# ctu-vras/trajectory_optimization

Hardware: AMD Instinct MI355X
Metric: point-visibility evals/sec (fwd+bwd) (higher is better)
Workload: dtype f32

## Files before the change

trajectory_optimization_amd/csrc/traj_kernels.hip:

```cpp
#include <algorithm>
#include <atomic>
#include <cstdlib>
#include <type_traits>

#include "common.hpp"
#include "opt_step.hpp"
#include "profile.hpp"

#define TO_SLOT 256
#define TO_TIE_CAP 7
#define TO_BWD_NSUM 14
#define TO_SP_THREADS 1024
#define TO_SP_WAVES (TO_SP_THREADS / 64)
#define TO_CBIT_STRIDE 16
#define TO_PROBE_MAXFW 1024
#define TO_SP_MAXW 1024
#define TO_PL_SHARDS 64
#define TO_PL_STRIDE 32

#ifdef TOHIP_STAMPS
#define TO_STAMP_BLOCKS 1024
#define TO_STAMP_N 12
enum { TO_STAMP_PROBE = 0, TO_STAMP_CULL, TO_STAMP_SPARSE, TO_STAMP_PAIRS, TO_STAMP_FINISH, TO_STAMP_KERNELS };
__device__ unsigned long long g_stamps[TO_STAMP_KERNELS][TO_STAMP_BLOCKS][TO_STAMP_N];
// ... 265 lines not shown
                const f2 p = vis_p_pk(r, k, f2{px[j], px[j + 1]}, f2{py[j], py[j + 1]}, f2{pz[j], pz[j + 1]}) *
                             f2{occ_one(occ, occw, v, (int64_t)sj0 * cv.sample_step), sj1 < cv.nsamples ? occ_one(occ, occw, v, (int64_t)sj1 * cv.sample_step) : 1.0f};
                mx = fmaxf(mx, p.x);
                mn = fminf(mn, p.x);
                if (sj1 < cv.nsamples) { mx = fmaxf(mx, p.y); mn = fminf(mn, p.y); }
            }
        }
    }
    for (int s = 32; s > 0; s >>= 1) { mx = fmaxf(mx, __shfl_xor(mx, s)); mn = fminf(mn, __shfl_xor(mn, s)); }
    if ((t & 63) == 0) { smx[t >> 6] = mx; smn[t >> 6] = mn; }
    __syncthreads();
    TO_STAMP(TO_STAMP_PROBE, 2);
    if (t == 0) {
        for (int w = 1; w < TO_PROBE_THREADS / 64; ++w) { mx = fmaxf(mx, smx[w]); mn = fminf(mn, smn[w]); }
        if (!(mn <= mx)) { mx = 0.f; mn = INFINITY; }
        const bool poisoned = cv.hdr[1] != 0;
        if (poisoned) { mx = __builtin_nanf(""); mn = INFINITY; }
        float thr, sthr;
        cull_bound(0.5f * mx, k.inv_var, &thr, &sthr);
        rec[v].Lh = (mn == 0.f && !poisoned) ? 0.49f * mx : 0.f;
        rec[v].L = mx;
        rec[v].U = mn;
        rec[v].thr1 = thr;
        rec[v].sthr1 = sthr;
        rec[v].azero = (mn == 0.f) ? 1.f : 0.f;
        scull[0] = thr; scull[1] = sthr; scull[2] = (mn == 0.f) ? 1.f : 0.f;
        Extrema e;
        e.nmn = -__builtin_bit_cast(int, mn);
        e.mx = __builtin_bit_cast(int, mx);
        e.pad[0] = e.pad[1] = 0;
        ext[v] = e;
        ties[v].nmax = 0;
        ties[v].nmin = 0;
    }
    TO_STAMP(TO_STAMP_PROBE, 3);
    if (!pc.on) return;
    __syncthreads();
    const float thr = scull[0], sthr = scull[1], azero = scull[2], inv_scd = 1.0f / k.scd;
    const int lane = t & 63;
    auto test_word = [&](int w, const float4& b) {
        const int sl = w * 64 + lane;
        const unsigned long long word = __ballot(sl < pc.nslots && tile_live(r.t, r.sp, thr, sthr, azero, b, inv_scd));
        if (lane == 0) pc.live[(int64_t)v * fv_words + w] = word;
    };
#pragma unroll
    for (int i = 0; i < kPre; ++i)
        if ((t >> 6) + i * kWaves < fv_words) test_word((t >> 6) + i * kWaves, tb[i]);
    for (int w0 = (t >> 6) + kPre * kWaves; w0 < fv_words; w0 += kPre * kWaves) {
#pragma unroll
        for (int i = 0; i < kPre; ++i) {
            const int sl = (w0 + i * kWaves) * 64 + lane;
            tb[i] = cv.bounds[sl < pc.nslots ? sl : 0];
        }
#pragma unroll
        for (int i = 0; i < kPre; ++i)
            if (w0 + i * kWaves < fv_words) test_word(w0 + i * kWaves, tb[i]);
    }
    TO_STAMP(TO_STAMP_PROBE, 4);
}


#define TO_P 4

__device__ __forceinline__ bool fold_extrema(Extrema* __restrict__ ext, int v, float mn, float mx, const WayRec& r) {
    bool cand = false;
    if (!(mx < r.Lh)) {
        cand = true;
        const int mxb = __builtin_bit_cast(int, mx);
        if (mxb > __builtin_bit_cast(int, r.L)) atomicMax(&ext[v].mx, mxb);
    }
    const int Ub = __builtin_bit_cast(int, r.U);
    if (Ub != 0) {
        const int mnb = __builtin_bit_cast(int, mn);
        if (mnb < Ub) atomicMax(&ext[v].nmn, -mnb);
    }
    return cand;
}

__device__ __forceinline__ unsigned long long* cbit_word(unsigned long long* cbits, int fv_words, int seg, int w) {
    return cbits + ((int64_t)seg * fv_words + w) * TO_CBIT_STRIDE;
}
__device__ __forceinline__ void mark_candidate(unsigned long long* __restrict__ cbits, int fv_words, int slot, int seg) {
    atomicOr(cbit_word(cbits, fv_words, seg, slot >> 6), 1ull << (slot & 63));
}

#define TO_PD 8
#define TO_DENSE_SGPRS 112
#define TO_DENSE_OCC_SGPRS 112
template <bool OCC>
__global__ void __launch_bounds__(TO_BLOCK)
k_traj_pass1_dense(CloudView cv, const WayRec* __restrict__ rec, int V, int nblk, EvalK k, float2* __restrict__ part,
                   Extrema* __restrict__ ext, unsigned long long* __restrict__ cbits, int fv_words,
                   const uint32_t* __restrict__ occ, int64_t occw, OutInit oi, unsigned long long* __restrict__ stamps) {
    constexpr int P = TO_PD;
    const int lane = threadIdx.x & 63;
    unsigned long long st0 = 0, sr0 = 0;
    if (stamps != nullptr && threadIdx.x == 0) { st0 = __builtin_amdgcn_s_memtime(); sr0 = __builtin_amdgcn_s_memrealtime(); }
    f2 eps2 = pk_splat(k.eps), l2e2 = pk_splat(k.l2e_eps), scd2 = pk_splat(k.scd);
    asm volatile("" : "+v"(eps2), "+v"(l2e2), "+v"(scd2));
    const int64_t total = (int64_t)nblk * V;
    int64_t u = total * blockIdx.x / gridDim.x;
    const int64_t u_end = total * (blockIdx.x + 1) / gridDim.x;
    const int64_t len = u_end - u, q1 = u + 3 * len / 4, q2 = u + 7 * len / 8, q3 = u + 15 * len / 16;
    __builtin_amdgcn_s_setprio(3);
    while (u < u_end) {
        const int pb = (int)(u / V);
        const int v0 = (int)(u - (int64_t)pb * V);
        const int v1 = (int)min((int64_t)V, v0 + (u_end - u));
        const int gthread = pb * TO_BLOCK + threadIdx.x;
        const int64_t base = (int64_t)gthread * P;
        const int slot = gthread >> 5;
        float x[P], y[P], z[P];
        load_points<P>(cv.soa, cv.npad, base, x, y, z);
        if (v0 == 0) { init_outputs(base, oi); init_outputs(base + 4, oi); }
        float2* prow = part + (int64_t)slot * V;
        for (int v = v0; v < v1; ++v) {
            const int64_t uu = u + (v - v0);
            if (uu == q1) __builtin_amdgcn_s_setprio(2);
            if (uu == q2) __builtin_amdgcn_s_setprio(1);
            if (uu == q3) __builtin_amdgcn_s_setprio(0);
            const WayRec& r = rec[v];
            float om[P];
            load_occ<P, OCC>(occ, occw, v, base, om);
            f2 p[P / 2];
#pragma unroll
            for (int i = 0; i < P; i += 2)
                p[i / 2] = vis_p_pk(r, k, f2{x[i], x[i + 1]}, f2{y[i], y[i + 1]}, f2{z[i], z[i + 1]}, eps2, l2e2, scd2) * f2{om[i], om[i + 1]};
            const float m1 = fmaxf(fmaxf(p[0].x, p[0].y), p[1].x), m2 = fmaxf(fmaxf(p[1].y, p[2].x), p[2].y);
            float mx = fmaxf(m2, fmaxf(fmaxf(p[3].x, p[3].y), m1));
            mx = half_max31_nn_fused(mx);
            float mn = 0.f;
            if (__builtin_bit_cast(int, r.U) != 0) {
                mn = fminf(fminf(fminf(p[0].x, p[0].y), fminf(p[1].x, p[1].y)), fminf(fminf(p[2].x, p[2].y), fminf(p[3].x, p[3].y)));
                mn = half_min31_nn_fused(mn);
            }
            if ((lane & 31) == 31) {
                prow[v] = make_float2(mn, mx);
                if (fold_extrema(ext, v, mn, mx, r)) mark_candidate(cbits, fv_words, slot, r.seg);
            }
        }
        u += v1 - v0;
    }
    if (stamps != nullptr && threadIdx.x == 0) {
        stamps[2 * blockIdx.x] = __builtin_amdgcn_s_memtime() - st0;
        stamps[2 * blockIdx.x + 1] = __builtin_amdgcn_s_memrealtime() - sr0;
        unsigned long long* ext_st = stamps + 2 * (int64_t)gridDim.x + 4 * (int64_t)blockIdx.x;
        unsigned hw, xcc;
        asm volatile("s_getreg_b32 %0, hwreg(HW_REG_HW_ID)" : "=s"(hw));
        asm volatile("s_getreg_b32 %0, hwreg(HW_REG_XCC_ID)" : "=s"(xcc));
        ext_st[0] = sr0; ext_st[1] = __builtin_amdgcn_s_memrealtime(); ext_st[2] = hw; ext_st[3] = xcc;
    }
}

__device__ __forceinline__ unsigned long long uniform_u64(unsigned long long v) {
    const unsigned lo = __builtin_amdgcn_readfirstlane((unsigned)v), hi = __builtin_amdgcn_readfirstlane((unsigned)(v >> 32));
    return ((unsigned long long)hi << 32) | lo;
}

#define TO_CULL_LIST 2048
struct CullLds {
    unsigned long long cand[TO_PROBE_MAXFW];
    unsigned long long row[TO_PROBE_MAXFW];
    int pre[TO_PROBE_MAXFW];
    int list[TO_CULL_LIST];
    int mx[2 * TO_SP_WAVES], mn[2 * TO_SP_WAVES];
    int total;
};

__device__ __forceinline__ int cull_select(const CullLds& L, int fv_words, int j, int lane) {
    int lo = 0, hi = fv_words;
    while (hi - lo > 1) {
        const int step = (hi - lo + 63) >> 6;
        const int idx = lo + lane * step;
        const int cnt = __popcll(__ballot(idx < hi && L.pre[idx] <= j));
        lo += (cnt - 1) * step;
        hi = min(hi, lo + step);
    }
    const unsigned long long word = uniform_u64(L.row[lo]);
    const int r = j - L.pre[lo];
    const bool hit = ((word >> lane) & 1ull) && __popcll(word & ((1ull << lane) - 1ull)) == r;
    return lo * 64 + __builtin_ctzll(__ballot(hit));
}

template <bool OCC, int NW>
__global__ void __launch_bounds__(NW * 64)
k_traj_pass1_cull(CloudView cv, const WayRec* __restrict__ rec, int V, EvalK k, float2* __restrict__ part, Extrema* __restrict__ ext,
                  unsigned long long* __restrict__ cbits, int fv_words, const unsigned long long* __restrict__ live,
                  const uint32_t* __restrict__ occ, int64_t occw, OutInit oi) {
    __shared__ CullLds L;
    const int t = threadIdx.x, lane = t & 63, wave = t >> 6;
    const int v = blockIdx.y;
    TO_STAMP(TO_STAMP_CULL, 0);
    for (int w = t; w < fv_words; w += NW * 64) { L.row[w] = live[(int64_t)v * fv_words + w]; L.cand[w] = 0ull; }
    if (oi.lo_zero != nullptr)
        for (int64_t i = (((int64_t)v * gridDim.x + blockIdx.x) * (NW * 64) + t) * 4; i < oi.npad; i += (int64_t)gridDim.y * gridDim.x * (NW * 64) * 4)
            init_outputs(i, oi);
    __syncthreads();
    TO_STAMP(TO_STAMP_CULL, 1);
    if (t < 64) {
        int carry = 0;
        for (int w0 = 0; w0 < fv_words; w0 += 64) {
            const int c = (w0 + lane < fv_words) ? __popcll(L.row[w0 + lane]) : 0;
            int incl = c;
#pragma unroll
            for (int sh = 1; sh < 64; sh <<= 1) {
                const int up = __shfl_up(incl, sh);
                if (lane >= sh) incl += up;
            }
            if (w0 + lane < fv_words) L.pre[w0 + lane] = carry + incl - c;
            carry += __shfl(incl, 63);
        }
        if (lane == 0) L.total = carry;
    }
    __syncthreads();
    const int n = L.total;
    const bool listed = n <= TO_CULL_LIST;
    if (listed) {
        for (int w = wave; w < fv_words; w += NW) {
            const unsigned long long word = L.row[w];
            if ((word >> lane) & 1ull) L.list[L.pre[w] + __popcll(word & ((1ull << lane) - 1ull))] = w * 64 + lane;
        }
        __syncthreads();
    }
    TO_STAMP(TO_STAMP_CULL, 2);
    const int wr = __builtin_amdgcn_readfirstlane((int)(blockIdx.x * NW) + wave), WR = (int)gridDim.x * NW;
    const WayRec& r = rec[v];
    int bmx = __builtin_bit_cast(int, r.L), bmn = __builtin_bit_cast(int, r.U);
    const int half = lane >> 5, nunits = (n + 1) >> 1;
    auto unit_slot = [&](int u) {
        if (listed) return L.list[min(2 * u + half, n - 1)];
        const int s0 = cull_select(L, fv_words, 2 * u, lane), s1 = cull_select(L, fv_words, min(2 * u + 1, n - 1), lane);
        return half ? s1 : s0;
    };
    if (wr < nunits) {
        constexpr int P8 = TO_PD;
        const f2 eps2 = pk_splat(k.eps), l2e2 = pk_splat(k.l2e_eps), scd2 = pk_splat(k.scd);
        auto eval_unit = [&](int u, int cur, const float (&x)[P8], const float (&y)[P8], const float (&z)[P8]) {
            const bool valid = 2 * u + half < n;
            float om[P8];
            load_occ<P8, OCC>(occ, occw, v, (int64_t)cur * TO_SLOT + (lane & 31) * P8, om);
            f2 p[P8 / 2];
#pragma unroll
            for (int i = 0; i < P8; i += 2)
                p[i / 2] = vis_p_pk(r, k, f2{x[i], x[i + 1]}, f2{y[i], y[i + 1]}, f2{z[i], z[i + 1]}, eps2, l2e2, scd2) * f2{om[i], om[i + 1]};
            const float m1 = fmaxf(fmaxf(p[0].x, p[0].y), p[1].x), m2 = fmaxf(fmaxf(p[1].y, p[2].x), p[2].y);
            const float mx = half_max31_nn_fused(fmaxf(m2, fmaxf(fmaxf(p[3].x, p[3].y), m1)));
            float mn = 0.f;
            if (__builtin_bit_cast(int, r.U) != 0) {
                mn = fminf(fminf(fminf(p[0].x, p[0].y), fminf(p[1].x, p[1].y)), fminf(fminf(p[2].x, p[2].y), fminf(p[3].x, p[3].y)));
                mn = half_min31_nn_fused(mn);
            }
            if ((lane & 31) == 31 && valid) {
                part[(int64_t)cur * V + v] = make_float2(mn, mx);
                if (!(mx < r.Lh)) {
                    atomicOr(&L.cand[cur >> 6], 1ull << (cur & 63));
                    bmx = max(bmx, __builtin_bit_cast(int, mx));
                }
                if (__builtin_bit_cast(int, r.U) != 0) bmn = min(bmn, __builtin_bit_cast(int, mn));
            }
        };
        float xa[P8], ya[P8], za[P8], xb[P8], yb[P8], zb[P8];
        int sa = unit_slot(wr), sb = 0;
        load_points<P8>(cv.soa, cv.npad, (int64_t)sa * TO_SLOT + (lane & 31) * P8, xa, ya, za);
        for (int u = wr; u < nunits; u += 2 * WR) {
            const bool more1 = u + WR < nunits, more2 = u + 2 * WR < nunits;
            if (more1) {
                sb = unit_slot(u + WR);
                load_points<P8>(cv.soa, cv.npad, (int64_t)sb * TO_SLOT + (lane & 31) * P8, xb, yb, zb);
            }
            eval_unit(u, sa, xa, ya, za);
            if (!more1) break;
            if (more2) {
                sa = unit_slot(u + 2 * WR);
                load_points<P8>(cv.soa, cv.npad, (int64_t)sa * TO_SLOT + (lane & 31) * P8, xa, ya, za);
            }
            eval_unit(u + WR, sb, xb, yb, zb);
        }
    }
    TO_STAMP(TO_STAMP_CULL, 3);
    if ((lane & 31) == 31) { L.mx[2 * wave + half] = bmx; L.mn[2 * wave + half] = bmn; }
    __syncthreads();
    TO_STAMP(TO_STAMP_CULL, 4);
    if (t == 0) {
        for (int w = 0; w < 2 * NW; ++w) { bmx = max(bmx, L.mx[w]); bmn = min(bmn, L.mn[w]); }
        if (bmx > __builtin_bit_cast(int, r.L)) atomicMax(&ext[v].mx, bmx);
        if (bmn < __builtin_bit_cast(int, r.U)) atomicMax(&ext[v].nmn, -bmn);
    }
    for (int w = t; w < fv_words; w += NW * 64) {
        const unsigned long long word = L.cand[w];
        if (word) atomicOr(cbit_word(cbits, fv_words, r.seg, w), word);
    }
    TO_STAMP(TO_STAMP_CULL, 5);
}


enum { TO_SP_FWD = 0, TO_SP_FUSED = 2 };
#define TO_SP_CW 4
#define TO_SP_STAGE (TO_SP_CW * 64)

struct SparseArgs {
    CloudView cv;
    const WayRec* rec;
    const Extrema* ext;
    EvalK k;
    const float2* part;
    int V, nslots, vwords, fv_words;
    const unsigned long long* cbits;
    const unsigned long long* live;
    int2* plist;
    int* npairs;
    int64_t plcap;
    unsigned long long* fv;
    TieRec* ties;
    float* lo_sum;
    float* minmax;
    const uint32_t* occ;
    int64_t occw;
    const int* toff;
    int n_traj, C;
    float* rewards;
    int prefilled;
    RewardAcc* acc;
    int shift;
    const float* grad_rewards;
    const float* scalars;
    const float* gout;
    float* bpart;
    float* unit;
};

struct __attribute__((aligned(16))) StagedWay {
    float t[3], f0[3], f1[3], f2[3], sp[3];
    float a, invM;
    int v;
    float pad[2];
};
static_assert(sizeof(StagedWay) == 80, "StagedWay is 20 floats");

template <int NW, int SFW>
struct SparseLds {
    unsigned long long sflag[SFW];
    StagedWay stage[TO_SP_STAGE];
    float4 spart[TO_SP_WAVES][64];
    int any[NW];
    int pbase;
};

__device__ __forceinline__ f2 log_odds_pk(const EvalK& k, float a, float invM, f2 p) {
    f2 ph = (p - pk_splat(a)) * pk_splat(invM);
    ph = f2{__builtin_amdgcn_fmed3f(ph.x, 0.5f, k.clip_hi), __builtin_amdgcn_fmed3f(ph.y, 0.5f, k.clip_hi)};
    const f2 om = pk_splat(1.0f) - ph;
    return (f2{to_log2(ph.x), to_log2(ph.y)} - f2{to_log2(om.x), to_log2(om.y)}) * pk_splat(0.693147180559945f);
}

__device__ __forceinline__ void stage_way(const SparseArgs& a, int v, StagedWay& dst) {
    const WayRec& r = a.rec[v];
    StagedWay sw;
    for (int i = 0; i < 3; ++i) { sw.t[i] = r.t[i]; sw.f0[i] = r.f0[i]; sw.f1[i] = r.f1[i]; sw.f2[i] = r.f2[i]; sw.sp[i] = r.sp[i]; }
    float pmax, M;
    load_norm(a.ext[v], sw.a, pmax, M, sw.invM);
    if (!(M > 0.f) || !(sw.invM < INFINITY)) sw.invM = __builtin_nanf("");
    sw.v = v;
    sw.pad[0] = sw.pad[1] = 0.f;
    dst = sw;
}

template <int MODE, bool OCC, int NW, int SFW>
__device__ __forceinline__ void sparse_slot(const SparseArgs& a, int slot, int tr, int acc_line, SparseLds<NW, SFW>& L) {
    constexpr int NSET = TO_SP_WAVES / NW;
    const int t = threadIdx.x, lane = t & 63, wave = t >> 6;
    TO_STAMP(TO_STAMP_SPARSE, 1);
    const EvalK& k = a.k;
    const int64_t base = (int64_t)slot * TO_SLOT + lane * 4;
    float x[4], y[4], z[4];
    load_points<4>(a.cv.soa, a.cv.npad, base, x, y, z);
    int4 o4 = make_int4(0, 0, 0, 0);
    if (MODE == TO_SP_FUSED && wave == 0) o4 = *reinterpret_cast<const int4*>(a.cv.perm + base);

    const int v_lo = a.toff ? a.toff[tr] * a.C : 0, v_hi = a.toff ? a.toff[tr + 1] * a.C : a.V;
    const int w_lo = v_lo >> 6, w_hi = min(a.vwords, (v_hi + 63) >> 6);
    const int wb = SFW < TO_SP_MAXW ? w_lo : 0;
    const bool direct = v_hi - v_lo <= TO_SP_STAGE;
    const bool stager = direct && t < v_hi - v_lo;
    StagedWay sw;
    if (stager) stage_way(a, v_lo + t, sw);
    int mine = 0;
    for (int w = w_lo + wave; w < w_hi; w += NW) {
        const int v = w * 64 + lane;
// ... 899 lines not shown
                                    uint32_t* rows, void* stream_) {
    if (!inv_perm || !kept_idx || !kept_count || !vis_idx || !vis_off || !all_visible || !rows || n <= 0 || n_wps <= 0 ||
        n_wps > 65535)
        return TOHIP_EINVAL;
    hipStream_t st = (hipStream_t)stream_;
    const int64_t npad = tohip_padded_points(n);
    const int64_t roww = npad / 32;
    hipError_t e = hipMemsetAsync(rows, 0xff, (size_t)roww * (size_t)n_wps * sizeof(uint32_t), st);
    if (e != hipSuccess) return (int)e;
    int nb = (int)((n + 255) / 256);
    if (nb > 256) nb = 256;
    const dim3 grid((unsigned)nb, (unsigned)n_wps);
    k_occ_rows_clear<<<grid, 256, 0, st>>>(inv_perm, kept_idx, n, kept_count, all_visible, rows, roww);
    TO_HIP_CHECK_LAUNCH();
    k_occ_rows_set<<<grid, 256, 0, st>>>(inv_perm, kept_idx, n, vis_idx, vis_off, all_visible, rows, roww);
    TO_HIP_CHECK_LAUNCH();
    k_occ_rows_pad<<<(int)((n_wps + 63) / 64), 64, 0, st>>>(n, npad, rows, roww, (int)n_wps);
    TO_HIP_CHECK_LAUNCH();
    return TOHIP_OK;
}

__global__ void k_occ_rows_masked(const int* __restrict__ inv, const int32_t* __restrict__ kept_idx, int64_t n,
                                  const int32_t* __restrict__ kept_count, const float* __restrict__ visible,
                                  const int64_t* __restrict__ seg_off, int min_points, uint32_t* __restrict__ rows, int64_t roww) {
    const int w = blockIdx.y;
    const int m = kept_count[w];
    if (m < min_points) return;
    const int32_t* kk = kept_idx + (int64_t)w * n;
    const float* vis = visible + seg_off[w];
    uint32_t* row = rows + (int64_t)w * roww;
    const int stride = gridDim.x * blockDim.x;
    if (inv != nullptr) {
        for (int j = blockIdx.x * blockDim.x + threadIdx.x; j < m; j += stride) {
            if (vis[j] == 0.f) {
                const int s = inv[kk[j]];
                atomicAnd(&row[s >> 5], ~(1u << (s & 31)));
            }
        }
        return;
    }
    const int lane = threadIdx.x & 63;
    for (int j0 = blockIdx.x * blockDim.x; j0 < m; j0 += stride) {
        const int j = j0 + threadIdx.x;
        int word = -1 - lane;
        unsigned bits = 0u;
        if (j < m && vis[j] == 0.f) { const int s = kk[j]; word = s >> 5; bits = 1u << (s & 31); }
        for (int d = 1; d < 64; d <<= 1) {
            const unsigned ob = (unsigned)__shfl_down((int)bits, d);
            const int ow = __shfl_down(word, d);
            if (lane + d < 64 && ow == word) bits |= ob;
        }
        const int pw = __shfl_up(word, 1);
        if (word >= 0 && (lane == 0 || pw != word)) atomicAnd(&row[word], ~bits);
    }
}

extern "C" int tohip_occlusion_rows_masked(int64_t n, const int32_t* inv_perm, const int32_t* kept_idx, const int32_t* kept_count,
                                           const float* visible, const int64_t* seg_off, int32_t min_points, int64_t n_wps, uint32_t* rows,
                                           void* stream_) {
    if (!kept_idx || !kept_count || !visible || !seg_off || !rows || n <= 0 || n_wps <= 0 || n_wps > 65535) return TOHIP_EINVAL;
    hipStream_t st = (hipStream_t)stream_;
    const int64_t npad = tohip_padded_points(n);
    const int64_t roww = npad / 32;
    hipError_t e = hipMemsetAsync(rows, 0xff, (size_t)roww * (size_t)n_wps * sizeof(uint32_t), st);
    if (e != hipSuccess) return (int)e;
    int nb = (int)((n + 255) / 256);
    if (nb > 256) nb = 256;
    k_occ_rows_masked<<<dim3((unsigned)nb, (unsigned)n_wps), 256, 0, st>>>(inv_perm, kept_idx, n, kept_count, visible, seg_off, min_points, rows, roww);
    TO_HIP_CHECK_LAUNCH();
    k_occ_rows_pad<<<(int)((n_wps + 63) / 64), 64, 0, st>>>(n, npad, rows, roww, (int)n_wps);
    TO_HIP_CHECK_LAUNCH();
    return TOHIP_OK;
}

extern "C" int tohip_inverse_permutation(const void* packed, int64_t n, int32_t* inv, void* stream_) {
    if (!packed || !inv || n <= 0) return TOHIP_EINVAL;
    const CloudView cv = cloud_view(packed, n);
    k_inverse_perm<<<(int)((n + 255) / 256), 256, 0, (hipStream_t)stream_>>>(cv.perm, n, inv);
    TO_HIP_CHECK_LAUNCH();
    return TOHIP_OK;
}

extern "C" int tohip_occlusion_row(int64_t n, const int32_t* inv_perm, const int32_t* kept_idx, const int32_t* kept_count,
                                   const int32_t* vis_idx, const int32_t* vis_count, uint32_t* row, void* stream_) {
    if (!inv_perm || !kept_idx || !kept_count || !vis_idx || !vis_count || !row || n <= 0) return TOHIP_EINVAL;
    hipStream_t st = (hipStream_t)stream_;
    const int64_t npad = tohip_padded_points(n);
    hipError_t e = hipMemsetAsync(row, 0xff, (size_t)(npad / 32) * sizeof(uint32_t), st);
    if (e != hipSuccess) return (int)e;
    int nb = (int)((n + 255) / 256);
    if (nb > 1024) nb = 1024;
    k_occ_clear_kept<<<nb, 256, 0, st>>>(inv_perm, kept_idx, kept_count, row);
    TO_HIP_CHECK_LAUNCH();
    k_occ_set_visible<<<nb, 256, 0, st>>>(inv_perm, kept_idx, vis_idx, vis_count, row);
    TO_HIP_CHECK_LAUNCH();
    k_occ_rows_pad<<<1, 64, 0, st>>>(n, npad, row, npad / 32, 1);
    TO_HIP_CHECK_LAUNCH();
    return TOHIP_OK;
}


namespace {

inline unsigned long long*& clock_stamps() { static unsigned long long* p = nullptr; return p; }

struct TrajPlan {
    int64_t npad;
    int nblk;
    int nslots;
    int ncbits;
    int fv_words;
    int vwords;
    int V;
    int64_t plcap;
    size_t off_ctl, off_toff, off_rec, off_cold, off_ext, off_cbits, off_ctr, off_part, off_fv, off_live, off_plist, off_ties, off_bpart, off_vgrad, off_unit, total;
};

inline TrajPlan make_plan(int64_t n, int64_t V, int64_t W, int64_t n_traj = 1) {
    TrajPlan p;
    p.npad = tohip_padded_points(n);
    p.nblk = (int)(p.npad / (TO_BLOCK * TO_P));
    p.nslots = (int)(p.npad / TO_SLOT);
    p.fv_words = (p.nslots + 63) / 64;
    p.ncbits = (int)((int64_t)p.fv_words * (n_traj < 1 ? 1 : n_traj));
    p.vwords = (int)((V + 63) / 64);
    p.V = (int)V;
    size_t o = 0;
    p.off_ctl = o;   o += sizeof(RewardAcc) * (size_t)(n_traj < 1 ? 1 : n_traj);
    p.off_toff = o;  o += align_up(sizeof(int) * (size_t)((n_traj < 1 ? 1 : n_traj) + 1), 256);
    p.off_rec = o;   o += align_up((size_t)V * sizeof(WayRec), 256);
    (void)W;
    p.off_cold = o;  o += align_up((size_t)V * sizeof(WayCold), 256);
    p.off_ext = o;   o += align_up((size_t)V * sizeof(Extrema), 256);
    p.off_cbits = o; o += align_up((size_t)p.ncbits * TO_CBIT_STRIDE * sizeof(unsigned long long), 256);
    p.off_ctr = o;   o += (size_t)TO_PL_SHARDS * TO_PL_STRIDE * sizeof(int);
    p.off_part = o;  o += align_up((size_t)V * (size_t)p.nslots * sizeof(float2), 256);
    p.off_fv = o;    o += align_up((size_t)V * (size_t)p.fv_words * sizeof(unsigned long long), 256);
    p.off_live = o;  o += align_up((size_t)V * (size_t)p.fv_words * sizeof(unsigned long long), 256);
    p.plcap = (int64_t)((p.nslots + TO_PL_SHARDS - 1) / TO_PL_SHARDS) * V;
    p.off_plist = o; o += align_up((size_t)p.plcap * TO_PL_SHARDS * sizeof(int2), 256);
    p.off_ties = o;  o += align_up((size_t)V * sizeof(TieRec), 256);
    p.off_bpart = o; o += align_up((size_t)V * (size_t)p.nslots * 16 * sizeof(float), 256);
    p.off_vgrad = o; o += align_up((size_t)V * 12 * sizeof(float), 256);
    p.off_unit = o;  o += align_up((size_t)n_traj * (size_t)p.npad * sizeof(float), 256);
    p.total = o;
    return p;
}

inline int dense_per_cu(int api, int sgprs) {
    const int by_sgpr = 800 / ((sgprs + 15) / 16 * 16 + 16);
    const int k = std::min(std::min(api, 8), by_sgpr);
    return k < 1 ? 1 : k;
}
inline int dense_blocks(int nblk, int V, bool occ) {
    constexpr int kDev = 64;
    static std::atomic<int> cache[kDev];
    int dev = 0;
    if (hipGetDevice(&dev) != hipSuccess) dev = -1;
    int e = (dev >= 0 && dev < kDev) ? cache[dev].load(std::memory_order_relaxed) : 0;
    if (e == 0) {
        int cus = 0;
        hipDeviceProp_t prop;
        if (dev >= 0 && hipGetDeviceProperties(&prop, dev) == hipSuccess) cus = prop.multiProcessorCount;
        if (cus <= 0) cus = 256;
        int a = 0, b = 0;
        if (hipOccupancyMaxActiveBlocksPerMultiprocessor(&a, k_traj_pass1_dense<false>, TO_BLOCK, 0) != hipSuccess || a <= 0) a = 4;
        if (hipOccupancyMaxActiveBlocksPerMultiprocessor(&b, k_traj_pass1_dense<true>, TO_BLOCK, 0) != hipSuccess || b <= 0) b = 4;
        e = cus << 8 | dense_per_cu(a, TO_DENSE_SGPRS) << 4 | dense_per_cu(b, TO_DENSE_OCC_SGPRS);
        if (dev >= 0 && dev < kDev) cache[dev].store(e, std::memory_order_relaxed);
    }
    const int cus = e >> 8, per_cu = occ ? (e & 15) : (e >> 4 & 15);
    int64_t nb = (int64_t)per_cu * cus;
    const int64_t total = (int64_t)nblk * V;
    if (nb > total) nb = total;
    return (int)nb;
}

inline int rig_cams(const tohip_rig* rig) { return (rig && rig->n_cams > 0 && rig->rig_quats) ? rig->n_cams : 1; }

struct TrajStep {
    hipStream_t st;
    TrajPlan pl;
    CloudView cv;
    EvalK k;
    int C;
    int64_t n, W, V, n_traj;
    const float *rq, *rt;
    const int* toff;
    int* toff_ws;
    const uint32_t* occ;
    int64_t occw;
    bool cull;
    int max_traj_v = 0;
    int wp_stride = 1;
    int traj_rows = 0;
    bool lean = false;
    OptStep opt = OptStep{};
    float* opt_scalars = nullptr;
    RewardAcc* acc;
    WayRec* rec;
    WayCold* cold;
    Extrema* ext;
    unsigned long long* cbits;
    int* ctr;
    int2* plist;
    float2* part;
    unsigned long long *fv, *live;
    TieRec* ties;
    float *bpart, *vgrad;
    float* unit;
    int shift;
};

inline int traj_step_init(TrajStep& s, const void* packed, int64_t n, int64_t W, int64_t n_traj, const int32_t* traj_offsets,
                          const tohip_camera* cam, const tohip_rig* rig, int flags, const uint32_t* occ, void* workspace,
                          size_t workspace_bytes, void* stream_, bool forward) {
    if (!packed || !cam || !workspace || n <= 0 || W <= 0 || n_traj <= 0 || n_traj > 65535 || (forward && n_traj > 1 && !traj_offsets)) return TOHIP_EINVAL;
    s.st = (hipStream_t)stream_;
    s.C = rig_cams(rig);
    s.n = n; s.W = W; s.V = W * s.C; s.n_traj = n_traj;
    if (s.V > 64 * TO_SP_MAXW || (int64_t)(tohip_padded_points(n) / TO_SLOT / 64 + 1) * n_traj > (int64_t)1 << 30) return TOHIP_EINVAL;
    s.pl = make_plan(n, s.V, W, n_traj);
    if (workspace_bytes < s.pl.total) return TOHIP_ENOSPC;
    char* ws = (char*)workspace;
    s.acc = (RewardAcc*)(ws + s.pl.off_ctl);
    s.rec = (WayRec*)(ws + s.pl.off_rec);
    s.cold = (WayCold*)(ws + s.pl.off_cold);
    s.ext = (Extrema*)(ws + s.pl.off_ext);
    s.cbits = (unsigned long long*)(ws + s.pl.off_cbits);
    s.ctr = (int*)(ws + s.pl.off_ctr);
    s.plist = (int2*)(ws + s.pl.off_plist);
    s.live = (unsigned long long*)(ws + s.pl.off_live);
    s.part = (float2*)(ws + s.pl.off_part);
    s.fv = (unsigned long long*)(ws + s.pl.off_fv);
    s.ties = (TieRec*)(ws + s.pl.off_ties);
    s.bpart = (float*)(ws + s.pl.off_bpart);
    s.vgrad = (float*)(ws + s.pl.off_vgrad);
    s.unit = (float*)(ws + s.pl.off_unit);
    s.k = make_evalk(cam);
    s.cv = cloud_view(packed, n);
    s.cull = !(flags & TOHIP_TRAJ_DENSE) && s.pl.fv_words <= TO_PROBE_MAXFW;
    s.wp_stride = ((flags >> 8) & 0xffff) + 1;
    if (s.wp_stride > 1 && n_traj > 1) return TOHIP_EINVAL;
    s.rq = (s.C > 1 || (rig && rig->rig_quats)) ? rig->rig_quats : nullptr;
    s.rt = s.rq ? rig->rig_trans : nullptr;
    s.toff_ws = (int*)(ws + s.pl.off_toff);
    s.toff = n_traj > 1 ? (forward ? traj_offsets : s.toff_ws) : nullptr;
    s.occ = occ;
    s.occw = s.cv.npad / 32;
    s.shift = reward_shift(n);
    return TOHIP_OK;
}

inline int launch_probe_pass1(const TrajStep& s, const float* poses, const float* quats, float* lo_sum, float* rewards_half) {
    const int V = (int)s.V;
    const OutInit oi{s.lean ? nullptr : lo_sum, s.lean ? nullptr : rewards_half, s.cv.npad, s.n, (int)s.n_traj};
    {
        TO_PROF(TOHIP_PROF_PROBE, s.st);
        const ProbeCull pc{s.cull ? 1 : 0, s.pl.nslots, s.live};
        const int grid = V;
        if (V <= 512)
            k_traj_probe<1024><<<grid, 1024, 0, s.st>>>(s.cv, poses, quats, s.C, s.rq, s.rt, s.k, s.rec, s.cold, s.ext, s.ties, s.occ, s.occw, s.fv,
                                                        s.pl.fv_words, s.acc, s.toff, s.toff_ws, (int)s.n_traj, s.cbits, s.pl.ncbits, s.ctr, s.wp_stride,
                                                        s.traj_rows, pc, V);
        else
            k_traj_probe<256><<<grid, 256, 0, s.st>>>(s.cv, poses, quats, s.C, s.rq, s.rt, s.k, s.rec, s.cold, s.ext, s.ties, s.occ, s.occw, s.fv,
                                                      s.pl.fv_words, s.acc, s.toff, s.toff_ws, (int)s.n_traj, s.cbits, s.pl.ncbits, s.ctr, s.wp_stride,
                                                      s.traj_rows, pc, V);
        TO_HIP_CHECK_LAUNCH();
    }
    {
        TO_PROF(TOHIP_PROF_PASS1, s.st);
        const bool occ = s.occ != nullptr;
        if (s.cull) {
            const dim3 grid(std::max(1, std::min(8, 1024 / V)), V);
            if (occ) k_traj_pass1_cull<true, 4><<<grid, 256, 0, s.st>>>(s.cv, s.rec, V, s.k, s.part, s.ext, s.cbits, s.pl.fv_words, s.live, s.occ, s.occw, oi);
            else k_traj_pass1_cull<false, 4><<<grid, 256, 0, s.st>>>(s.cv, s.rec, V, s.k, s.part, s.ext, s.cbits, s.pl.fv_words, s.live, s.occ, s.occw, oi);
        } else {
            const int nblk8 = (int)(s.pl.npad / (TO_BLOCK * TO_PD));
            const int nb = dense_blocks(nblk8, V, occ);
            if (occ) k_traj_pass1_dense<true><<<nb, TO_BLOCK, 0, s.st>>>(s.cv, s.rec, V, nblk8, s.k, s.part, s.ext, s.cbits, s.pl.fv_words, s.occ, s.occw, oi, clock_stamps());
            else k_traj_pass1_dense<false><<<nb, TO_BLOCK, 0, s.st>>>(s.cv, s.rec, V, nblk8, s.k, s.part, s.ext, s.cbits, s.pl.fv_words, s.occ, s.occw, oi, clock_stamps());
        }
        TO_HIP_CHECK_LAUNCH();
    }
    return TOHIP_OK;
}

inline SparseArgs sparse_args(const TrajStep& s, float* lo_sum) {
    SparseArgs a;
    a.cv = s.cv; a.rec = s.rec; a.ext = s.ext; a.k = s.k; a.part = s.part;
    a.V = (int)s.V; a.nslots = s.pl.nslots; a.vwords = s.pl.vwords; a.fv_words = s.pl.fv_words; a.cbits = s.cbits; a.live = s.cull ? s.live : nullptr; a.plist = s.plist; a.npairs = s.ctr; a.plcap = s.pl.plcap;
    a.fv = s.fv; a.ties = s.ties; a.lo_sum = lo_sum; a.minmax = nullptr; a.occ = s.occ; a.occw = s.occw;
    a.toff = s.toff; a.n_traj = (int)s.n_traj; a.C = s.C;
    a.rewards = nullptr; a.prefilled = 0; a.acc = s.acc; a.shift = s.shift;
    a.grad_rewards = nullptr; a.scalars = nullptr; a.gout = nullptr; a.bpart = s.bpart; a.unit = s.unit;
    return a;
}

constexpr int kSparseWaves = 4;
inline int pair_blocks() {
    static const int cus = [] {
        int dev = 0;
        hipDeviceProp_t prop;
        if (hipGetDevice(&dev) == hipSuccess && hipGetDeviceProperties(&prop, dev) == hipSuccess && prop.multiProcessorCount > 0) return prop.multiProcessorCount;
        return 256;
    }();
    return cus;
}

inline bool sparse_small_flags(const TrajStep& s) {
    if (s.n_traj == 1) return s.V <= 8 * 64;
    return s.max_traj_v > 0 && s.max_traj_v <= 7 * 64;
}
inline int sparse_blocks(const TrajStep& s) {
    const int64_t resident = (int64_t)pair_blocks() * (sparse_small_flags(s) ? 4 : 3);
    const int64_t per_traj = std::max<int64_t>(1, std::min<int64_t>(s.pl.nslots, resident / s.n_traj));
    return (int)(per_traj * s.n_traj);
}

template <int MODE, bool OCC>
inline void launch_sparse_occ(const TrajStep& s, const SparseArgs& a) {
    constexpr int NW = kSparseWaves;
    const int grid = sparse_blocks(s) + (s.opt.mode ? s.opt.n_traj : 0);
    if (sparse_small_flags(s)) k_traj_sparse<MODE, OCC, NW, 8><<<grid, NW * 64, 0, s.st>>>(a, s.opt);
    else k_traj_sparse<MODE, OCC, NW, TO_SP_MAXW><<<grid, NW * 64, 0, s.st>>>(a, s.opt);
}

template <int MODE>
inline int launch_sparse(const TrajStep& s, const SparseArgs& a) {
    if (s.occ) launch_sparse_occ<MODE, true>(s, a);
    else launch_sparse_occ<MODE, false>(s, a);
    TO_HIP_CHECK_LAUNCH();
    return TOHIP_OK;
}

inline int launch_pairs(const TrajStep& s, const SparseArgs& a) {
    const int grid = pair_blocks() + (s.opt.mode == 2 ? 1 : 0);
    const bool unit = a.unit != nullptr && a.grad_rewards == nullptr && a.scalars == nullptr;
    if (s.occ) {
        if (unit) k_traj_pairs<true, true><<<grid, TO_SP_THREADS, 0, s.st>>>(a, s.opt, s.opt_scalars);
        else k_traj_pairs<true, false><<<grid, TO_SP_THREADS, 0, s.st>>>(a, s.opt, s.opt_scalars);
    } else {
        if (unit) k_traj_pairs<false, true><<<grid, TO_SP_THREADS, 0, s.st>>>(a, s.opt, s.opt_scalars);
        else k_traj_pairs<false, false><<<grid, TO_SP_THREADS, 0, s.st>>>(a, s.opt, s.opt_scalars);
    }
    TO_HIP_CHECK_LAUNCH();
    return TOHIP_OK;
}

inline int launch_finish(const TrajStep& s, const FinishPost& post, float* poses_grad, float* quats_grad) {
    TO_PROF(TOHIP_PROF_FINISH, s.st);
    const bool single = s.C == 1 && s.rq == nullptr;
    const int V = (int)s.V;
    if (V <= 512)
        k_traj_finish<1024><<<V, 1024, 0, s.st>>>(s.cv, s.bpart, s.pl.nslots, s.fv, s.pl.fv_words, s.rec, s.ext, s.k, s.ties, s.part, V, s.occ, s.occw,
                                                  s.vgrad, s.cold, single ? 1 : 0, poses_grad, quats_grad, post, s.opt);
    else
        k_traj_finish<256><<<V, 256, 0, s.st>>>(s.cv, s.bpart, s.pl.nslots, s.fv, s.pl.fv_words, s.rec, s.ext, s.k, s.ties, s.part, V, s.occ, s.occw,
                                                s.vgrad, s.cold, single ? 1 : 0, poses_grad, quats_grad, post, s.opt);
    TO_HIP_CHECK_LAUNCH();
    if (!single && post.mode != 3) {
        k_traj_bwd_finish2<<<(int)((s.W + 63) / 64), 64, 0, s.st>>>(s.vgrad, s.rec, s.cold, (int)s.W, s.C, s.rq, s.rt, poses_grad, quats_grad, s.opt,
                                                                    post.scalars_out);
        TO_HIP_CHECK_LAUNCH();
    }
    return TOHIP_OK;
}

inline FinishPost finish_post(const TrajStep& s, int mode, const float* scalars, const float* gout, float* scalars_out, float eps) {
    FinishPost p;
    p.live = s.cull ? s.live : nullptr;
    p.partial = nullptr;
    p.mode = mode; p.scalars = scalars; p.gout = gout; p.acc = s.acc; p.scalars_out = scalars_out; p.n = s.n; p.shift = s.shift; p.eps = eps;
    p.toff = s.toff; p.C = s.C;
    return p;
}

inline int reward_blocks(int64_t n) {
    int64_t nb = (n + 4 * TO_SP_THREADS - 1) / (4 * TO_SP_THREADS);
    return (int)(nb > TO_REWARD_BLOCKS ? TO_REWARD_BLOCKS : nb);
}

}

extern "C" size_t tohip_traj_workspace_bytes_multi(int64_t n_points, int64_t n_virtual, int64_t n_traj) {
    if (n_points <= 0 || n_virtual <= 0 || n_traj <= 0) return 0;
    return make_plan(n_points, n_virtual, n_virtual, n_traj).total;
}
extern "C" size_t tohip_traj_workspace_bytes(int64_t n_points, int64_t n_virtual) {
    return tohip_traj_workspace_bytes_multi(n_points, n_virtual, 1);
}

extern "C" int tohip_traj_forward_multi(const void* packed, int64_t n, const float* poses, const float* quats, int64_t W,
                                        const int32_t* traj_offsets, int64_t n_traj, const tohip_camera* cam, const tohip_rig* rig,
                                        int flags, const uint32_t* occlusion_bits, float* lo_sum, float* minmax, float* rewards_half,
                                        void* workspace, size_t workspace_bytes, void* stream_) {
    if (!poses || !quats || !lo_sum || !minmax) return TOHIP_EINVAL;
    TrajStep s;
    int rc = traj_step_init(s, packed, n, W, n_traj, traj_offsets, cam, rig, flags, occlusion_bits, workspace, workspace_bytes, stream_, true);
    if (rc != TOHIP_OK) return rc;
    rc = launch_probe_pass1(s, poses, quats, lo_sum, rewards_half);
    if (rc != TOHIP_OK) return rc;
    TO_PROF(TOHIP_PROF_PASS2, s.st);
    SparseArgs a = sparse_args(s, lo_sum);
    a.minmax = minmax;
    return launch_sparse<TO_SP_FWD>(s, a);
}

extern "C" int tohip_traj_forward(const void* packed, int64_t n, const float* poses, const float* quats, int64_t W,
                                  const tohip_camera* cam, const tohip_rig* rig, int flags, const uint32_t* occlusion_bits,
                                  float* lo_sum, float* minmax, float* rewards_half, void* workspace, size_t workspace_bytes,
                                  void* stream_) {
    return tohip_traj_forward_multi(packed, n, poses, quats, W, nullptr, 1, cam, rig, flags, occlusion_bits, lo_sum, minmax, rewards_half,
                                    workspace, workspace_bytes, stream_);
}

extern "C" int tohip_traj_reward_multi(const void* packed, const float* lo_sum, int64_t n, int64_t n_traj, float eps, int prefilled,
                                       float* rewards, float* scalars, void* workspace, size_t workspace_bytes, void* stream_) {
    if (!packed || !lo_sum || !rewards || !scalars || !workspace || n <= 0 || n_traj <= 0 || n_traj > 65535) return TOHIP_EINVAL;
    hipStream_t st = (hipStream_t)stream_;
    if (workspace_bytes < sizeof(RewardAcc) * (size_t)n_traj) return TOHIP_ENOSPC;
    RewardAcc* acc = (RewardAcc*)workspace;
    const CloudView cv = cloud_view(packed, n);
    TO_PROF(TOHIP_PROF_REWARD, st);
    k_traj_reward<<<dim3(reward_blocks(n), (unsigned)n_traj), TO_SP_THREADS, 0, st>>>(lo_sum, cv.perm, n, cv.npad, eps, reward_shift(n), prefilled ? 1 : 0,
                                                                                 rewards, acc, scalars);
    TO_HIP_CHECK_LAUNCH();
    return TOHIP_OK;
}

extern "C" int tohip_traj_reward(const void* packed, const float* lo_sum, int64_t n, float eps, int prefilled, float* rewards,
                                 float* scalars, void* workspace, size_t workspace_bytes, void* stream_) {
    return tohip_traj_reward_multi(packed, lo_sum, n, 1, eps, prefilled, rewards, scalars, workspace, workspace_bytes, stream_);
}
// ... 275 lines not shown
extern "C" int tohip_traj_pshard_local(const void* packed, int64_t n_local, int64_t n_global, int64_t W, const tohip_camera* cam,
                                       const tohip_rig* rig, int flags, const uint32_t* occlusion_bits, float* lo_sum, float* minmax,
                                       float* rewards, double* partial, void* workspace, size_t workspace_bytes, void* stream_) {
    if (!lo_sum || !minmax || !rewards || !partial || n_global < n_local) return TOHIP_EINVAL;
    TrajStep s;
    int rc = traj_step_init(s, packed, n_local, W, 1, nullptr, cam, rig, flags, occlusion_bits, workspace, workspace_bytes, stream_, false);
    if (rc != TOHIP_OK) return rc;
    s.shift = reward_shift(n_global);
    SparseArgs a = sparse_args(s, lo_sum);
    a.minmax = minmax;
    a.rewards = rewards;
    a.prefilled = 1;
    rc = launch_sparse<TO_SP_FUSED>(s, a);
    if (rc != TOHIP_OK) return rc;
    rc = launch_pairs(s, a);
    if (rc != TOHIP_OK) return rc;
    FinishPost post = finish_post(s, 3, nullptr, nullptr, nullptr, cam->eps);
    post.partial = partial;
    return launch_finish(s, post, nullptr, nullptr);
}

extern "C" int tohip_traj_pshard_finish(int64_t n_local, int64_t n_global, int64_t W, const tohip_camera* cam, const tohip_rig* rig,
                                        const double* partial, const float* gout, float* scalars, float* poses_grad, float* quats_grad,
                                        void* workspace, size_t workspace_bytes, void* stream_) {
    if (!cam || !partial || !scalars || !poses_grad || !quats_grad || !workspace || n_local <= 0 || n_global < n_local || W <= 0) return TOHIP_EINVAL;
    const int C = rig_cams(rig);
    const int64_t V = W * C;
    const TrajPlan pl = make_plan(n_local, V, W, 1);
    if (workspace_bytes < pl.total) return TOHIP_ENOSPC;
    hipStream_t st = (hipStream_t)stream_;
    char* ws = (char*)workspace;
    const WayRec* rec = (const WayRec*)(ws + pl.off_rec);
    const WayCold* cold = (const WayCold*)(ws + pl.off_cold);
    float* vgrad = (float*)(ws + pl.off_vgrad);
    const bool single = C == 1 && !(rig && rig->rig_quats);
    k_traj_pshard_final<<<(int)V, 64, 0, st>>>(partial, rec, (const Extrema*)(ws + pl.off_ext), cold, single ? 1 : 0, reward_shift(n_global), cam->eps,
                                               gout, scalars, vgrad, poses_grad, quats_grad);
    TO_HIP_CHECK_LAUNCH();
    if (!single) {
        k_traj_bwd_finish2<<<(int)((W + 63) / 64), 64, 0, st>>>(vgrad, rec, cold, (int)W, C, rig->rig_quats, rig->rig_trans, poses_grad, quats_grad,
                                                                OptStep{}, nullptr);
        TO_HIP_CHECK_LAUNCH();
    }
    return TOHIP_OK;
}


__global__ void k_candidate_flags(const unsigned long long* __restrict__ cbits, int fv_words, int n_traj, int nslots, int* __restrict__ flag) {
    for (int sl = blockIdx.x * blockDim.x + threadIdx.x; sl < nslots; sl += gridDim.x * blockDim.x) {
        unsigned long long any = 0ull;
        for (int tr = 0; tr < n_traj; ++tr) any |= cbits[((int64_t)tr * fv_words + (sl >> 6)) * TO_CBIT_STRIDE];
        flag[sl] = (int)((any >> (sl & 63)) & 1ull);
    }
}

__global__ void __launch_bounds__(1024) k_flag_prefix(const int* __restrict__ flag, int nslots, int* __restrict__ prefix) {
    __shared__ int part[1024];
    const int t = threadIdx.x;
    const int per = (nslots + 1023) / 1024;
    int c = 0;
    for (int j = 0; j < per; ++j) { const int s = t * per + j; if (s < nslots) c += flag[s] != 0; }
    part[t] = c;
    __syncthreads();
    for (int d = 1; d < 1024; d <<= 1) {
        const int v = t >= d ? part[t - d] : 0;
        __syncthreads();
        part[t] += v;
        __syncthreads();
    }
    int run = t ? part[t - 1] : 0;
    for (int j = 0; j < per; ++j) {
        const int s = t * per + j;
        if (s < nslots) { prefix[s] = run; run += flag[s] != 0; }
    }
    if (t == 1023) prefix[nslots] = part[1023];
}

__global__ void __launch_bounds__(TO_SLOT)
k_slots_move(const int* __restrict__ flag, const int* __restrict__ prefix, int nslots, float* __restrict__ lo_sum,
             float* __restrict__ compact, int64_t capacity_slots, int pack) {
    for (int s = blockIdx.x; s < nslots; s += gridDim.x) {
        if (!flag[s]) continue;
        const int e = prefix[s];
        if (e >= capacity_slots) continue;
        if (pack) compact[(int64_t)e * TO_SLOT + threadIdx.x] = lo_sum[(int64_t)s * TO_SLOT + threadIdx.x];
        else lo_sum[(int64_t)s * TO_SLOT + threadIdx.x] = compact[(int64_t)e * TO_SLOT + threadIdx.x];
    }
}

extern "C" int tohip_traj_candidate_flags(int64_t n_points, int64_t n_virtual, int64_t n_traj, const void* workspace, size_t workspace_bytes,
                                          int32_t* slot_flags, void* stream_) {
    if (n_points <= 0 || n_virtual <= 0 || n_traj <= 0 || !workspace || !slot_flags) return TOHIP_EINVAL;
    const TrajPlan pl = make_plan(n_points, n_virtual, n_virtual, n_traj);
    if (workspace_bytes < pl.total) return TOHIP_ENOSPC;
    hipStream_t st = (hipStream_t)stream_;
    const char* ws = (const char*)workspace;
    k_candidate_flags<<<16, 256, 0, st>>>((const unsigned long long*)(ws + pl.off_cbits), pl.fv_words, (int)n_traj, pl.nslots, slot_flags);
    TO_HIP_CHECK_LAUNCH();
    return TOHIP_OK;
}

extern "C" int tohip_slot_flags_prefix(const int32_t* slot_flags, int64_t n_points, int32_t* prefix, void* stream_) {
    if (!slot_flags || !prefix || n_points <= 0) return TOHIP_EINVAL;
    const int nslots = (int)(tohip_padded_points(n_points) / TO_SLOT);
    k_flag_prefix<<<1, 1024, 0, (hipStream_t)stream_>>>(slot_flags, nslots, prefix);
    TO_HIP_CHECK_LAUNCH();
    return TOHIP_OK;
}

extern "C" int tohip_slots_pack(const int32_t* slot_flags, const int32_t* prefix, int64_t n_points, float* lo_sum, float* compact,
                                int64_t capacity_slots, int pack, void* stream_) {
    if (!slot_flags || !prefix || !lo_sum || !compact || n_points <= 0 || capacity_slots < 0) return TOHIP_EINVAL;
    const int nslots = (int)(tohip_padded_points(n_points) / TO_SLOT);
    k_slots_move<<<nslots < 2048 ? nslots : 2048, TO_SLOT, 0, (hipStream_t)stream_>>>(slot_flags, prefix, nslots, lo_sum, compact, capacity_slots, pack);
    TO_HIP_CHECK_LAUNCH();
    return TOHIP_OK;
}

__global__ void k_traj_stats(const unsigned long long* __restrict__ cbits, int ncbits, const int* __restrict__ ctr, int nslots, int V,
                             const unsigned long long* __restrict__ live, int nlive_words, unsigned long long* __restrict__ stats) {
    unsigned long long c = 0, e = 0;
    for (int i = threadIdx.x; i < ncbits; i += blockDim.x) c += __popcll(cbits[(int64_t)i * TO_CBIT_STRIDE]);
    for (int i = threadIdx.x; i < nlive_words; i += blockDim.x) e += (unsigned long long)__popcll(live[i]);
    for (int s = 32; s > 0; s >>= 1) { c += __shfl_xor(c, s); e += __shfl_xor(e, s); }
    if ((threadIdx.x & 63) == 0 && c) atomicAdd(&stats[1], c);
    if ((threadIdx.x & 63) == 0 && e) atomicAdd(&stats[4], e);
    if (threadIdx.x == 0) {
        unsigned long long np = 0;
        for (int l = 0; l < TO_PL_SHARDS; ++l) np += (unsigned long long)ctr[l * TO_PL_STRIDE];
        stats[0] = np;
    }
    if (threadIdx.x == 0) { stats[2] = (unsigned long long)nslots; stats[3] = (unsigned long long)V; }
}

extern "C" int tohip_traj_step_stats(int64_t n_points, int64_t n_virtual, int64_t n_traj, const void* workspace, size_t workspace_bytes,
                                     int64_t* stats, void* stream_) {
    if (n_points <= 0 || n_virtual <= 0 || n_traj <= 0 || !workspace || !stats) return TOHIP_EINVAL;
    const TrajPlan pl = make_plan(n_points, n_virtual, n_virtual, n_traj);
    if (workspace_bytes < pl.total) return TOHIP_ENOSPC;
    const char* ws = (const char*)workspace;
    k_traj_stats<<<1, 1024, 0, (hipStream_t)stream_>>>((const unsigned long long*)(ws + pl.off_cbits), pl.ncbits, (const int*)(ws + pl.off_ctr), pl.nslots,
                                                       (int)n_virtual, (const unsigned long long*)(ws + pl.off_live), (int)(n_virtual * pl.fv_words), (unsigned long long*)stats);
    TO_HIP_CHECK_LAUNCH();
    return TOHIP_OK;
}

extern "C" int tohip_profile_clock(void* buffer) {
    clock_stamps() = (unsigned long long*)buffer;
    return TOHIP_OK;
}
extern "C" int64_t tohip_profile_clock_blocks(int64_t n_points, int64_t n_virtual, int flags, int with_occlusion) {
    if (n_points <= 0 || n_virtual <= 0 || !(flags & TOHIP_TRAJ_DENSE)) return 0;
    const TrajPlan pl = make_plan(n_points, n_virtual, n_virtual);
    const int nblk8 = (int)(pl.npad / (TO_BLOCK * TO_PD));
    return dense_blocks(nblk8, (int)n_virtual, with_occlusion != 0);
}
```

Before: 1002 billion.

## Add 16-points-per-thread dense pass1 kernel with XCD-aware block mapping

Adds a wide dense pass-1 kernel in which each thread evaluates 16 points per waypoint instead of 8, so 16 lanes form a slot row. Per-point loads, waypoint record reads and reduction overhead are amortised over more work. Blocks are remapped so contiguous work pieces land on the same CU within each XCD, and wave priority is lowered in steps as a block nears the end of its range. The wide path is chosen only without occlusion and when there are enough units for every resident block. In exchange it uses more registers and lowers occupancy to three blocks per CU, and it pins the cull kernel to an explicit 8-point constant.

```diff
diff --git a/trajectory_optimization_amd/csrc/traj_kernels.hip b/trajectory_optimization_amd/csrc/traj_kernels.hip
--- a/trajectory_optimization_amd/csrc/traj_kernels.hip
+++ b/trajectory_optimization_amd/csrc/traj_kernels.hip
@@ -441,12 +441,95 @@
     }
 }
 
+#define TO_PD16 16
+#define TO_XCDS 8
+#define TO_WIDE_SGPRS 112
+#define TO_WIDE_MIN_UNITS 2
+template <bool OCC>
+__global__ void __launch_bounds__(TO_BLOCK, 3)
+k_traj_pass1_dense16(CloudView cv, const WayRec* __restrict__ rec, int V, int nblk, EvalK k, float2* __restrict__ part,
+                     Extrema* __restrict__ ext, unsigned long long* __restrict__ cbits, int fv_words,
+                     const uint32_t* __restrict__ occ, int64_t occw, OutInit oi, unsigned long long* __restrict__ stamps, int per_cu) {
+    constexpr int P = TO_PD16;
+    const int lane = threadIdx.x & 63;
+    unsigned long long st0 = 0, sr0 = 0;
+    if (stamps != nullptr && threadIdx.x == 0) { st0 = __builtin_amdgcn_s_memtime(); sr0 = __builtin_amdgcn_s_memrealtime(); }
+    f2 eps2 = pk_splat(k.eps), l2e2 = pk_splat(k.l2e_eps), scd2 = pk_splat(k.scd);
+    asm volatile("" : "+v"(eps2), "+v"(l2e2), "+v"(scd2));
+    int piece = blockIdx.x;
+    if (per_cu > 0) {
+        const int per_xcd = gridDim.x / TO_XCDS, cus = per_xcd / per_cu, j = blockIdx.x / TO_XCDS;
+        piece = (blockIdx.x % TO_XCDS) * per_xcd + (j % cus) * per_cu + j / cus;
+    }
+    const int64_t total = (int64_t)nblk * V;
+    int64_t u = total * piece / gridDim.x;
+    const int64_t u_end = total * (piece + 1) / gridDim.x;
+    const int64_t len = u_end - u, q1 = u + 3 * len / 4, q2 = u + 7 * len / 8, q3 = u + 15 * len / 16;
+    __builtin_amdgcn_s_setprio(3);
+    while (u < u_end) {
+        const int pb = (int)(u / V);
+        const int v0 = (int)(u - (int64_t)pb * V);
+        const int v1 = (int)min((int64_t)V, v0 + (u_end - u));
+        const int gthread = pb * TO_BLOCK + threadIdx.x;
+        const int64_t base = (int64_t)gthread * P;
+        const bool present = base < cv.npad;
+        const int64_t lbase = present ? base : 0;
+        const int slot = gthread >> 4;
+        float x[P], y[P], z[P];
+        load_points<P>(cv.soa, cv.npad, lbase, x, y, z);
+        if (v0 == 0 && present) {
+#pragma unroll
+            for (int j = 0; j < P; j += 4) init_outputs(base + j, oi);
+        }
+        float2* prow = part + (int64_t)slot * V;
+        for (int v = v0; v < v1; ++v) {
+            const int64_t uu = u + (v - v0);
+            if (uu == q1) __builtin_amdgcn_s_setprio(2);
+            if (uu == q2) __builtin_amdgcn_s_setprio(1);
+            if (uu == q3) __builtin_amdgcn_s_setprio(0);
+            const WayRec& r = rec[v];
+            float om[P];
+            load_occ<P, OCC>(occ, occw, v, lbase, om);
+            f2 p[P / 2];
+#pragma unroll
+            for (int i = 0; i < P; i += 2)
+                p[i / 2] = vis_p_pk(r, k, f2{x[i], x[i + 1]}, f2{y[i], y[i + 1]}, f2{z[i], z[i + 1]}, eps2, l2e2, scd2) * f2{om[i], om[i + 1]};
+            const float a0 = fmaxf(fmaxf(p[0].x, p[0].y), p[1].x), a1 = fmaxf(fmaxf(p[1].y, p[2].x), p[2].y),
+                        a2 = fmaxf(fmaxf(p[3].x, p[3].y), p[4].x), a3 = fmaxf(fmaxf(p[4].y, p[5].x), p[5].y),
+                        a4 = fmaxf(fmaxf(p[6].x, p[6].y), p[7].x);
+            const float mx = row_max16_nn(fmaxf(fmaxf(fmaxf(a0, a1), a2), fmaxf(fmaxf(a3, a4), p[7].y)));
+            float mn = 0.f;
+            if (__builtin_bit_cast(int, r.U) != 0) {
+                float m = fminf(p[0].x, p[0].y);
+#pragma unroll
+                for (int i = 1; i < P / 2; ++i) m = fminf(m, fminf(p[i].x, p[i].y));
+                mn = row_min16_nn(m);
+            }
+            if ((lane & 15) == 15 && present) {
+                prow[v] = make_float2(mn, mx);
+                if (fold_extrema(ext, v, mn, mx, r)) mark_candidate(cbits, fv_words, slot, r.seg);
+            }
+        }
+        u += v1 - v0;
+    }
+    if (stamps != nullptr && threadIdx.x == 0) {
+        stamps[2 * blockIdx.x] = __builtin_amdgcn_s_memtime() - st0;
+        stamps[2 * blockIdx.x + 1] = __builtin_amdgcn_s_memrealtime() - sr0;
+        unsigned long long* ext_st = stamps + 2 * (int64_t)gridDim.x + 4 * (int64_t)blockIdx.x;
+        unsigned hw, xcc;
+        asm volatile("s_getreg_b32 %0, hwreg(HW_REG_HW_ID)" : "=s"(hw));
+        asm volatile("s_getreg_b32 %0, hwreg(HW_REG_XCC_ID)" : "=s"(xcc));
+        ext_st[0] = sr0; ext_st[1] = __builtin_amdgcn_s_memrealtime(); ext_st[2] = hw; ext_st[3] = xcc | 0x100u;
+    }
+}
+
 __device__ __forceinline__ unsigned long long uniform_u64(unsigned long long v) {
     const unsigned lo = __builtin_amdgcn_readfirstlane((unsigned)v), hi = __builtin_amdgcn_readfirstlane((unsigned)(v >> 32));
     return ((unsigned long long)hi << 32) | lo;
 }
 
 #define TO_CULL_LIST 2048
+#define TO_CULL_PD 8
 struct CullLds {
     unsigned long long cand[TO_PROBE_MAXFW];
     unsigned long long row[TO_PROBE_MAXFW];
@@ -522,7 +605,7 @@
         return half ? s1 : s0;
     };
     if (wr < nunits) {
-        constexpr int P8 = TO_PD;
+        constexpr int P8 = TO_CULL_PD;
         const f2 eps2 = pk_splat(k.eps), l2e2 = pk_splat(k.l2e_eps), scd2 = pk_splat(k.scd);
         auto eval_unit = [&](int u, int cur, const float (&x)[P8], const float (&y)[P8], const float (&z)[P8]) {
             const bool valid = 2 * u + half < n;
@@ -1728,7 +1811,13 @@
     const int k = std::min(std::min(api, 8), by_sgpr);
     return k < 1 ? 1 : k;
 }
-inline int dense_blocks(int nblk, int V, bool occ) {
+struct DenseLaunch {
+    bool wide;
+    int nblk;
+    int nb;
+    int per_cu;
+};
+inline DenseLaunch dense_blocks(int64_t npad, int V, bool occ) {
     constexpr int kDev = 64;
     static std::atomic<int> cache[kDev];
     int dev = 0;
@@ -1739,17 +1828,23 @@
         hipDeviceProp_t prop;
         if (dev >= 0 && hipGetDeviceProperties(&prop, dev) == hipSuccess) cus = prop.multiProcessorCount;
         if (cus <= 0) cus = 256;
-        int a = 0, b = 0;
+        int a = 0, b = 0, w = 0;
         if (hipOccupancyMaxActiveBlocksPerMultiprocessor(&a, k_traj_pass1_dense<false>, TO_BLOCK, 0) != hipSuccess || a <= 0) a = 4;
         if (hipOccupancyMaxActiveBlocksPerMultiprocessor(&b, k_traj_pass1_dense<true>, TO_BLOCK, 0) != hipSuccess || b <= 0) b = 4;
-        e = cus << 8 | dense_per_cu(a, TO_DENSE_SGPRS) << 4 | dense_per_cu(b, TO_DENSE_OCC_SGPRS);
+        if (hipOccupancyMaxActiveBlocksPerMultiprocessor(&w, k_traj_pass1_dense16<false>, TO_BLOCK, 0) != hipSuccess || w <= 0) w = 2;
+        e = cus << 12 | dense_per_cu(w, TO_WIDE_SGPRS) << 8 | dense_per_cu(a, TO_DENSE_SGPRS) << 4 | dense_per_cu(b, TO_DENSE_OCC_SGPRS);
         if (dev >= 0 && dev < kDev) cache[dev].store(e, std::memory_order_relaxed);
     }
-    const int cus = e >> 8, per_cu = occ ? (e & 15) : (e >> 4 & 15);
-    int64_t nb = (int64_t)per_cu * cus;
-    const int64_t total = (int64_t)nblk * V;
-    if (nb > total) nb = total;
-    return (int)nb;
+    const int cus = e >> 12;
+    const int64_t nblk16 = (npad + TO_BLOCK * TO_PD16 - 1) / (TO_BLOCK * TO_PD16), resident16 = (int64_t)(e >> 8 & 15) * cus;
+    DenseLaunch d;
+    d.per_cu = 0;
+    d.wide = !occ && nblk16 * V >= TO_WIDE_MIN_UNITS * resident16;
+    d.nblk = d.wide ? (int)nblk16 : (int)(npad / (TO_BLOCK * TO_PD));
+    const int64_t resident = d.wide ? resident16 : (int64_t)(occ ? (e & 15) : (e >> 4 & 15)) * cus;
+    d.nb = (int)std::min(resident, (int64_t)d.nblk * V);
+    if (d.wide && d.nb == resident && cus % TO_XCDS == 0) d.per_cu = e >> 8 & 15;
+    return d;
 }
 
 inline int rig_cams(const tohip_rig* rig) { return (rig && rig->n_cams > 0 && rig->rig_quats) ? rig->n_cams : 1; }
@@ -1853,10 +1948,10 @@
             if (occ) k_traj_pass1_cull<true, 4><<<grid, 256, 0, s.st>>>(s.cv, s.rec, V, s.k, s.part, s.ext, s.cbits, s.pl.fv_words, s.live, s.occ, s.occw, oi);
             else k_traj_pass1_cull<false, 4><<<grid, 256, 0, s.st>>>(s.cv, s.rec, V, s.k, s.part, s.ext, s.cbits, s.pl.fv_words, s.live, s.occ, s.occw, oi);
         } else {
-            const int nblk8 = (int)(s.pl.npad / (TO_BLOCK * TO_PD));
-            const int nb = dense_blocks(nblk8, V, occ);
-            if (occ) k_traj_pass1_dense<true><<<nb, TO_BLOCK, 0, s.st>>>(s.cv, s.rec, V, nblk8, s.k, s.part, s.ext, s.cbits, s.pl.fv_words, s.occ, s.occw, oi, clock_stamps());
-            else k_traj_pass1_dense<false><<<nb, TO_BLOCK, 0, s.st>>>(s.cv, s.rec, V, nblk8, s.k, s.part, s.ext, s.cbits, s.pl.fv_words, s.occ, s.occw, oi, clock_stamps());
+            const DenseLaunch d = dense_blocks(s.pl.npad, V, occ);
+            if (d.wide) k_traj_pass1_dense16<false><<<d.nb, TO_BLOCK, 0, s.st>>>(s.cv, s.rec, V, d.nblk, s.k, s.part, s.ext, s.cbits, s.pl.fv_words, s.occ, s.occw, oi, clock_stamps(), d.per_cu);
+            else if (occ) k_traj_pass1_dense<true><<<d.nb, TO_BLOCK, 0, s.st>>>(s.cv, s.rec, V, d.nblk, s.k, s.part, s.ext, s.cbits, s.pl.fv_words, s.occ, s.occw, oi, clock_stamps());
+            else k_traj_pass1_dense<false><<<d.nb, TO_BLOCK, 0, s.st>>>(s.cv, s.rec, V, d.nblk, s.k, s.part, s.ext, s.cbits, s.pl.fv_words, s.occ, s.occw, oi, clock_stamps());
         }
         TO_HIP_CHECK_LAUNCH();
     }
@@ -2438,6 +2533,5 @@
 extern "C" int64_t tohip_profile_clock_blocks(int64_t n_points, int64_t n_virtual, int flags, int with_occlusion) {
     if (n_points <= 0 || n_virtual <= 0 || !(flags & TOHIP_TRAJ_DENSE)) return 0;
     const TrajPlan pl = make_plan(n_points, n_virtual, n_virtual);
-    const int nblk8 = (int)(pl.npad / (TO_BLOCK * TO_PD));
-    return dense_blocks(nblk8, (int)n_virtual, with_occlusion != 0);
-}
+    return dense_blocks(pl.npad, (int)n_virtual, with_occlusion != 0).nb;
+}
```

Measured after the change: 1031 billion (median of 6 runs). 1.03x the previous value.
